# sun-huangqingbo/multiplexed-image-annotator

Measured on AMD Instinct MI355X. Metric: cells/sec annotated (whole node), higher is better.
Workload: dtype f16

## Files before the change

multiplexed-image-annotator_amd/_lib.py:

```python
from __future__ import annotations

import ctypes
import os
from ctypes import POINTER, c_char_p, c_double, c_float, c_int32, c_int64, c_uint32, c_uint64, c_void_p

HERE = os.path.dirname(os.path.abspath(__file__))
LIB_PATH = os.path.join(HERE, "libribca_hip.so")
if os.environ.get("RIBCA_LIB"):
    LIB_PATH = os.environ["RIBCA_LIB"] if os.path.isabs(os.environ["RIBCA_LIB"]) else os.path.join(HERE, os.environ["RIBCA_LIB"])

TEST_LIB_PATH = LIB_PATH[:-3] + "_test.so"

_lib = None
_test_lib = None

SIGNATURES = {
    "ribca_version": (c_int32, []),
    "ribca_last_error": (c_char_p, []),
    "ribca_mask_minmax": (c_int32, [c_void_p, c_int64, c_void_p, c_void_p]),
    "ribca_label_table": (c_int32, [c_void_p, c_int32, c_int32, c_int32, c_void_p, c_void_p, c_void_p]),
    "ribca_channel_min": (c_int32, [c_void_p, c_int32, c_int64, c_void_p, c_void_p]),
    "ribca_extract_patches": (c_int32, [c_void_p, c_int32, c_int32, c_int32, c_void_p, c_void_p, c_void_p, c_void_p, c_void_p, c_int32,
                                        c_void_p, c_void_p, c_void_p]),
    "ribca_extract_patches_scaled": (c_int32, [c_void_p, c_int32, c_int32, c_int32, c_void_p, c_void_p, c_void_p, c_void_p, c_void_p, c_int32,
# ... 148 lines not shown
                                            c_void_p, c_int32, c_void_p]),
    "ribca_test_gemm_fold": (c_int32, [c_int32, c_void_p, c_int32, c_void_p, c_int32, c_int32, c_int32, c_int32, c_void_p, c_void_p,
                                       c_void_p, c_void_p, c_int32, c_void_p]),
    "ribca_test_qkv_attention_fold": (c_int32, [c_void_p, c_int32, c_void_p, c_int32, c_int32, c_int32, c_int32, c_void_p, c_void_p,
                                                c_void_p, c_void_p, c_void_p, c_void_p, c_void_p, c_int32, c_void_p]),
    "ribca_test_gemm_duo_gelu": (c_int32, [c_void_p, c_int32, c_void_p, c_int32, c_int32, c_int32, c_int32, c_void_p, c_void_p, c_void_p,
                                           c_void_p, c_void_p, c_int32, c_void_p]),
    "ribca_test_cell_attention": (c_int32, [c_void_p, c_int32, c_void_p, c_int32, c_int32, c_int32, c_void_p, c_void_p, c_void_p, c_void_p, c_int32,
                                            c_void_p]),
    "ribca_test_cell_mlp_image_bytes": (c_int64, [c_int32]),
    "ribca_test_cell_mlp": (c_int32, [c_void_p, c_int32, c_void_p, c_void_p, c_void_p, c_void_p, c_void_p, c_void_p, c_void_p, c_void_p, c_int32,
                                      c_void_p, c_int32, c_void_p, c_int32, c_int32, c_void_p]),
    "ribca_test_cls_attention_cell_tile": (c_int32, []),
    "ribca_test_cls_attention": (c_int32, [c_void_p, c_int32, c_void_p, c_int32, c_void_p, c_void_p, c_int32, c_int32, c_void_p, c_void_p, c_void_p,
                                           c_int32, c_void_p]),
    "ribca_test_qkv_attention_tokens": (c_int32, [c_int32, c_void_p, c_int32, c_void_p, c_int32, c_int32, c_int32, c_int32, c_int32, c_int32, c_void_p,
                                                  c_void_p, c_void_p, c_void_p, c_void_p, c_void_p, c_void_p, c_int32, c_void_p]),
    "ribca_test_attention_v_elems": (c_int64, [c_int32, c_int32, c_int32, c_int32]),
    "ribca_gemm_padded_n": (c_int32, [c_int32]),
}


class RibcaError(RuntimeError):
    pass


class _Library:

    def __init__(self, handle):
        self._handle = handle
# ... 72 lines not shown
```

multiplexed-image-annotator_amd/build.py:

```python
from __future__ import annotations

import concurrent.futures
import os
import subprocess
import sys

HERE = os.path.dirname(os.path.abspath(__file__))
CSRC = os.path.join(HERE, "csrc")
LIB = os.path.join(HERE, "libribca_hip.so")
LIB_TEST = os.path.join(HERE, "libribca_hip_test.so")
TEST_SOURCES = ["ribca_test_api.hip"]
EXPORTS = os.path.join(CSRC, "exports.map")
SOURCES = ["gemm_split16.hip", "gemm_duo.hip", "gemm_mx.hip", "attention.hip", "cell_attention.hip", "cell_mlp.hip", "cls_attention.hip", "vit_misc.hip", "preprocess.hip", "preprocess_scaled.hip", "vote.hip", "colorize.hip", "knn.hip", "umap.hip", "hdbscan.hip", "regions.hip", "spectral.hip", "scatter.hip", "celltype_stats.hip", "perm.hip", "enrichment.hip", "autocorr.hip", "local_autocorr.hip", "cooccurrence.hip", "nearest.hip", "contact.hip", "morphology.hip", "intensities.hip", "expand.hip", "components.hip", "outlines.hip", "overlap.hip", "localization.hip", "normalize.hip", "ribca_api.hip"]
HEADERS = ["ribca_common.h", "ribca_kernels.h", "ribca_scratch.h", "ribca_perm.h", "ribca_rowtable.h", "ribca_cellbox.h", "ribca_status.h", "ribca_internal.h", "gemm_epi.h", os.path.join("..", "..", "include", "ribca_hip.h"),
           os.path.join("..", "..", "include", "ribca_hip_test.h")]
FLAGS = ["-O3", "--offload-arch=gfx950", "-fPIC", "-std=c++17", "-Wall", "-Wno-unused-function", "-fvisibility=hidden", "-fvisibility-inlines-hidden",
         "-fno-slp-vectorize"]


def source_fingerprint() -> str:
    import hashlib
    h = hashlib.sha256()
    for name in sorted(SOURCES + TEST_SOURCES) + sorted(HEADERS):
        path = os.path.normpath(os.path.join(CSRC, name))
        h.update(os.path.basename(path).encode() + b"\0")
        with open(path, "rb") as f:
            h.update(f.read())
    h.update(" ".join(FLAGS).encode())
# ... 60 lines not shown
```

multiplexed-image-annotator_amd/csrc/ribca_api.hip:

```cpp
#include <hip/hip_runtime.h>

#include <cmath>
#include <cstdarg>
#include <cstdlib>
#include <cstdio>
#include <cstring>
#include <string>
#include <vector>

#include "../../include/ribca_hip.h"
#include "ribca_common.h"
#include "ribca_internal.h"
#include "ribca_kernels.h"
#include "ribca_scratch.h"
#include "ribca_status.h"

using namespace ribca;

namespace {

int fail(const std::string& msg) { return api_fail(msg.c_str()); }
int hip_fail(hipError_t e, const char* what) { return api_hip_fail(e, what); }

inline int round_up(int v, int m) { return (v + m - 1) / m * m; }
// ... 69 lines not shown
}

struct BlockW {
  const float *ln1w, *ln1b, *qkvb, *projb, *ln2w, *ln2b, *fc1b, *fc2b;
  const uint16_t *qkvw, *projw, *fc1w, *fc2w;
  const uint16_t* qkvwf = nullptr;
  const uint16_t* fc1wf;
  const uint16_t *projwf = nullptr, *fc2wf = nullptr;
  const float *qkvc = nullptr, *qkvb2 = nullptr, *fc1c = nullptr, *fc1b2 = nullptr;
  const uint16_t* fc2mxh = nullptr; const unsigned char* fc2mxx = nullptr;
  const uint16_t *qkvmxh = nullptr, *fc1mxh = nullptr; const unsigned char *qkvmxx = nullptr, *fc1mxx = nullptr;
  const uint16_t* mlpimg = nullptr;
};

bool env_on(const char* name) { return !(getenv(name) && atoi(getenv(name)) == 0); }
struct Switches { bool mx, mxz, cell_attn, cell_mlp, cls_attn; };
const Switches& switches() {
  static const Switches sw = {env_on("RIBCA_MX"), env_on("RIBCA_MXZ"), env_on("RIBCA_CELL_ATTN"), env_on("RIBCA_CELL_MLP"), env_on("RIBCA_CLS_ATTN")};
  return sw;
}
bool mx_on(int D) { return switches().mx && (4 * D) % 128 == 0 && gemm_mx_supported(D, 4 * D); }
bool mx_z_on(int D) { return switches().mxz && mx_on(D) && D % 192 == 0; }

struct BlockPath {
  bool fold, mx_fc2, mx_z, cell_attn, cell_mlp, cls_attn;
  BlockPath precise() const { return {fold, false, false, cell_attn, cell_mlp, cls_attn}; }
  bool qkv_mx3() const { return mx_z && !cell_attn; }
  bool qkv_buffers() const { return !(cell_attn && cls_attn); }
};
BlockPath block_path(const AttnGeom& a, bool fold) {
  const bool cell_attn = fold && switches().cell_attn && cell_attention_supported(a.D, a.H, a.T);
  return {fold, fold && mx_on(a.D), fold && mx_z_on(a.D), cell_attn, cell_attn && switches().cell_mlp && cell_mlp_supported(a.D),
          fold && switches().cls_attn && cls_attention_supported(a.D, a.H, a.T)};
}

struct ribca_vit {
  int D, C, K, depth, Dp;
  BlockPath path;
  char* arena = nullptr;
  size_t arena_bytes = 0;
  const float *cls, *pos, *pe_b, *norm_w, *norm_b, *head_w, *head_b;
  const float* pe_w;
  std::vector<BlockW> layers;
};

struct ribca_mae {
  int L, enc_depth, dec_depth;
  BlockPath enc_path, dec_path;
// ... 113 lines not shown
      launch_mx_pack_w(L.fc1w, 2 * Dp, 4 * D, Dp, Kz, const_cast<uint16_t*>(L.fc1mxh), const_cast<unsigned char*>(L.fc1mxx), s);
    }
    if (path.cell_mlp) launch_cell_mlp_pack(L.projw, L.fc1w, L.fc2w, D, const_cast<uint16_t*>(L.mlpimg), s);
  }
};
int64_t block_params(int64_t d) { return 2 * d + 3 * d * d + 3 * d + d * d + d + 2 * d + 4 * d * d + 4 * d + 4 * d * d + d; }

struct BlockWs {
  float* z; uint16_t* xa; uint16_t* q; uint16_t* k; uint16_t* vt; uint16_t* h;
  size_t qk_bytes, vt_bytes, xa_bytes;
  uint16_t* zps = nullptr; float2* part = nullptr; float2* rs = nullptr;
  MxAct zmx = MxAct{nullptr, nullptr, nullptr, 0, 0};
  size_t zmx_rows = 0;
  float *cls_g = nullptr, *cls_y = nullptr;
};
BlockWs carve_blocks(Carver& c, int cells, const AttnGeom& a, const BlockPath& p) {
  BlockWs w;
  const size_t Mc = (size_t)cells * a.T;
  const int Dp = round_up(a.D, 32);
  if (p.fold) {
    w.z = nullptr;
    w.zps = c.take<uint16_t>(Mc * 2 * Dp);
    w.part = c.take<float2>((p.cell_mlp ? (size_t)cells : Mc) * gemm_resid_part_rows(a.D));
    w.rs = c.take<float2>(Mc);
    if (p.mx_z) {
      const int Kz = round_up(a.D, 128);
      w.zmx.hi = c.take<uint16_t>(Mc * Kz);
      w.zmx.l8 = c.take<unsigned char>(Mc * Kz);
      w.zmx.sc = c.take<unsigned char>(Mc * (Kz / 32));
      w.zmx.Kp = Kz;
      w.zmx_rows = Mc;
    }
  } else {
    w.z = c.take<float>(Mc * a.D);
  }
  w.xa_bytes = Mc * 2 * Dp * sizeof(uint16_t);
  w.xa = c.take<uint16_t>(Mc * 2 * Dp);
  w.q = w.k = w.vt = nullptr;
  w.qk_bytes = w.vt_bytes = 0;
  if (p.qkv_buffers()) {
    const size_t qk = (size_t)cells * a.H * a.TP * 2 * a.hdq;
    w.qk_bytes = qk * sizeof(uint16_t);
    w.q = c.take<uint16_t>(qk);
    w.k = c.take<uint16_t>(qk);
    const size_t vt = attention_v_elems(a, cells);
    w.vt_bytes = vt * sizeof(uint16_t);
    w.vt = c.take<uint16_t>(vt);
  }
  const size_t cls_elems = p.cls_attn ? cls_attention_scratch_elems(cells, a.D) : 0;
  if (p.cls_attn && !p.qkv_buffers()) {
    w.cls_g = c.take<float>(cls_elems);
    w.cls_y = c.take<float>(cls_elems);
  }
  w.h = c.take<uint16_t>((p.cell_mlp ? (size_t)cells : Mc) * 2 * 4 * a.D);
  if (p.cls_attn && p.qkv_buffers()) {
    w.cls_g = reinterpret_cast<float*>(w.h);
    w.cls_y = w.cls_g + cls_elems;
  }
  return w;
}
int zero_pads(const BlockWs& w, const BlockPath& p, hipStream_t s) {
  HIP_TRY(hipMemsetAsync(w.xa, 0, w.xa_bytes, s));
  if (p.fold) HIP_TRY(hipMemsetAsync(w.zps, 0, w.xa_bytes, s));
  if (p.qkv_buffers()) {
    HIP_TRY(hipMemsetAsync(w.q, 0, w.qk_bytes, s));
    HIP_TRY(hipMemsetAsync(w.k, 0, w.qk_bytes, s));
    HIP_TRY(hipMemsetAsync(w.vt, 0, w.vt_bytes, s));
  }
  if (p.mx_z) {
// ... 88 lines not shown
      launch_ln_finalize(w.part, sg.tiles, Mc, sg.bn, D, w.rs, s);
    }
    return;
  }
  {
    ProfScope ps(P_FC1, s);
    GemmArgs g{w.zps, ld_x, L.fc1w, ld_x, Mc, 4 * D, Dp, L.fc1b2, L.fc1wf};
    launch_gemm_gelu_ln(g, w.rs, L.fc1c, w.h, ld_h, s);
  }
  {
    ProfScope ps(P_FC2, s);
    GemmArgs g{w.h, ld_h, L.fc2w, ld_h, Mc, D, 4 * D, L.fc2b, L.fc2wf};
    resid_ps_and_stats(g, w, ld_x, D, true, 1, s);
  }
}
void run_last_block_cls_fold(const BlockW& L, const BlockWs& w, int cells, const AttnGeom& a, const BlockPath& p, hipStream_t s) {
  const int D = a.D, Dp = round_up(D, 32), ld_x = 2 * Dp, ld_h = 2 * 4 * D, Mc = cells * a.T;
  const float scale = 1.0f / sqrtf((float)a.hd);
  if (p.cls_attn) {
    { ProfScope ps(P_QKV, s); launch_cls_attn_qg(w.zps, ld_x, L.qkvw, ld_x, L.qkvb2, w.rs, cells, D, scale, w.cls_g, s); }
    {
      ProfScope ps(P_ATTN, s);
      launch_cls_attn_ybar(w.zps, ld_x, w.rs, w.cls_g, cells, D, w.cls_y, s);
      launch_cls_attn_out(w.cls_y, L.qkvw, ld_x, L.qkvb2, cells, D, w.xa, ld_x, s);
    }
  } else {
    {
      ProfScope ps(P_QKV, s);
      GemmArgs gkv{w.zps, ld_x, L.qkvw + (size_t)D * ld_x, ld_x, Mc, 2 * D, Dp, L.qkvb2 + D};
      launch_gemm_qkv_ln(gkv, w.rs, L.qkvc + D, w.q, w.k, w.vt, a, scale, s, D, 0, 1);
      GemmArgs gq{w.zps, a.T * ld_x, L.qkvw, ld_x, cells, D, Dp, L.qkvb2};
      launch_gemm_qkv_ln(gq, w.rs, L.qkvc, w.q, w.k, w.vt, a, scale, s, 0, 1, a.T);
    }
    { ProfScope ps(P_ATTN, s); launch_attention(w.q, w.k, w.vt, w.xa, ld_x, cells, a, s, 1); }
  }
  {
    ProfScope ps(P_PROJ, s);
    GemmArgs g{w.xa, a.T * ld_x, L.projw, ld_x, cells, D, Dp, L.projb};
    resid_ps_and_stats(g, w, a.T * ld_x, D, true, a.T, s);
// ... 36 lines not shown
  const int64_t d = D;
  return d + (int64_t)kTokens * d + d * C * 16 + d + (int64_t)depth * block_params(d) + 2 * d + (int64_t)K * d + K;
}

int ribca_vit_create(const float* blob, int64_t blob_len, int32_t D, int32_t C, int32_t K, int32_t depth, void* stream, ribca_vit_t** out) {
  if (!out) return fail("ribca_vit_create: out is NULL");
  *out = nullptr;
  if (D <= 0 || D % 48 != 0 || D > 768) return fail("ribca_vit_create: D must be a multiple of 48 and <= 768");
  if (C <= 0 || C > 64 || K <= 0 || K > 16 || depth <= 0) return fail("ribca_vit_create: bad C/K/depth");
  if (!attention_supported(make_attn_geom(D, kHeads, kTokens))) return fail("ribca_vit_create: unsupported head dimension");
  if (blob_len != ribca_vit_blob_len(D, C, K, depth)) return fail("ribca_vit_create: blob length does not match (D, C, K, depth)");
  hipStream_t s = (hipStream_t)stream;
  ribca_vit* m = new ribca_vit();
  m->D = D; m->C = C; m->K = K; m->depth = depth;
  m->Dp = round_up(D, 32);
  m->path = block_path(make_attn_geom(D, kHeads, kTokens), true);
  m->arena_bytes = layout(m, nullptr);
  hipError_t e = hipMalloc((void**)&m->arena, m->arena_bytes);
  if (e != hipSuccess) { delete m; return hip_fail(e, "hipMalloc(weights)"); }
  layout(m, m->arena);
  BlobReader r{blob, s};
  r.copy(m->cls, D);
  r.copy(m->pos, (size_t)kTokens * D);
  r.copy(m->pe_w, (size_t)D * 16 * C);
  r.copy(m->pe_b, D);
  for (auto& L : m->layers) r.block(L, D, m->path);
  r.copy(m->norm_w, D); r.copy(m->norm_b, D);
  r.copy(m->head_w, (size_t)K * D); r.copy(m->head_b, K);
  e = r.err != hipSuccess ? r.err : hipGetLastError();
  if (e != hipSuccess) { ribca_vit_destroy(m); return hip_fail(e, "weight packing"); }
  if (api_finish() != 0) { ribca_vit_destroy(m); return 1; }
// ... 44 lines not shown
      ProfScope ps(P_EMBED, s);
      launch_embed_ps(patches + (size_t)c0 * c_img * 1600, c_img, src_chan, m->C, m->pe_w, m->pe_b, m->pos, w.zps, ld_z, D, bc, s);
    }
    {
      ProfScope ps(P_OTHER, s);
      launch_cls_rows_ps(w.zps, ld_z, m->cls, m->pos, D, bc, kTokens, s);
    }
    { ProfScope ps(P_LN, s); launch_row_stats_ps(w.zps, ld_z, bc * kTokens, D, w.rs, true, s); }
    if (path.qkv_mx3() && n_whole > 0) {
      ProfScope ps(P_OTHER, s);
      MxAct zmx = w.zmx;
      zmx.M = bc * kTokens;
      launch_mx_pack_act(w.zps, ld_z, bc * kTokens, m->Dp, zmx, s);
    }
    for (size_t li = 0; li < n_whole; ++li) run_block_fold(m->layers[li], w, bc, geom, path, path.qkv_mx3() && li + 1 < n_whole, s);
    run_last_block_cls_fold(m->layers.back(), w, bc, geom, path, s);
    {
      ProfScope ps(P_HEAD, s);
      launch_head_softmax_ps(w.zps, ld_z, m->norm_w, m->norm_b, m->head_w, m->head_b, probs + (size_t)c0 * m->K, D, m->K, bc, s);
    }
  }
  RIBCA_FINISH();
  return 0;
}
int ribca_vit_forward(const ribca_vit_t* m, const float* patches, int32_t c_img, const int32_t* src_chan, int32_t n_cells, float* probs,
                      void* workspace, int64_t workspace_bytes, int32_t chunk_cells, void* stream) {
  if (!m) return fail("ribca_vit_forward: model is NULL");
  return vit_forward_impl(m, m->path, patches, c_img, src_chan, n_cells, probs, workspace, workspace_bytes, chunk_cells, stream);
}
int ribca_vit_forward_precise(const ribca_vit_t* m, const float* patches, int32_t c_img, const int32_t* src_chan, int32_t n_cells, float* probs,
                              void* workspace, int64_t workspace_bytes, int32_t chunk_cells, void* stream) {
  if (!m) return fail("ribca_vit_forward: model is NULL");
// ... 379 lines not shown
```

multiplexed-image-annotator_amd/csrc/ribca_internal.h:

```cpp
#pragma once
#include <stdint.h>

#include "ribca_kernels.h"
#include "ribca_status.h"

#define RIBCA_INTERNAL_VERSION 6005

#define RIBCA_INTERNAL_FUNCS(X)                                                                                                              \
  X(api_finish) X(api_fail) X(mx_wh_bytes) X(mx_wx_bytes) X(gemm_padded_n) X(gemm_resid_bn) X(gemm_resid_tiles) X(gemm_resid_part_rows)      \
  X(gemm_mx_supported) X(cell_attention_supported) X(make_attn_geom) X(launch_pack_wf)                                                      \
  X(launch_pack_weight) X(launch_pack_weight_fold) X(launch_mx_pack_w) X(launch_mx_pack_act) X(launch_layernorm_ps) X(launch_row_stats_ps)   \
  X(launch_ln_finalize) X(launch_gemm_resid) X(launch_gemm_gelu) X(launch_gemm_qkv) X(launch_gemm_qkv_ln) X(launch_gemm_gelu_ln)             \
  X(launch_gemm_gelu_mx) X(launch_gemm_resid_ps) X(launch_gemm_mx_resid) X(launch_gemm_mx_qkv_ln) X(launch_gemm_mx_gelu) X(launch_attention) \
  X(launch_cell_qkv_attention) X(cell_mlp_supported) X(cell_mlp_image_bytes) X(launch_cell_mlp_pack) X(launch_cell_mlp)                     \
  X(cls_attention_supported) X(cls_attention_cell_tile) X(launch_cls_attn_qg) X(launch_cls_attn_ybar) X(launch_cls_attn_out)           \
  X(attention_supported) X(attention_v_elems)

namespace ribca {
struct InternalTable {
  int32_t version;
  int32_t n_funcs;
#define RIBCA_X(name) decltype(&ribca::name) name;
  RIBCA_INTERNAL_FUNCS(RIBCA_X)
#undef RIBCA_X
};
}
```

multiplexed-image-annotator_amd/csrc/ribca_kernels.h:

```cpp
#pragma once
#include <hip/hip_runtime.h>
#include <stdint.h>

namespace ribca {

int gemm_pick_bn(int N);
int gemm_padded_n(int N);

struct GemmArgs {
  const uint16_t* A; int lda;
  const uint16_t* W; int ldw;
  int M, N, Kp;
  const float* bias;
  const uint16_t* WF = nullptr;
};
void launch_pack_wf(const uint16_t* W, int ldw, int Np, int Kp, uint16_t* WF, hipStream_t s);
void launch_gemm_resid(const GemmArgs& g, float* z, int ldz, hipStream_t s);
void launch_gemm_gelu(const GemmArgs& g, uint16_t* out, int ldo, hipStream_t s);
struct ResidStatGeom { int tiles, bn; };
struct MxAct { uint16_t* hi; unsigned char* l8; unsigned char* sc; int Kp; int M; };
ResidStatGeom launch_gemm_resid_ps(const GemmArgs& g, uint16_t* z, int ldz, float2* part, const float2* prev, int prev_stride, hipStream_t s,
                                   bool force_duo = false, const MxAct* zmx = nullptr);
int gemm_resid_tiles(int N);
int gemm_resid_bn(int N);
// ... 35 lines not shown
                               uint16_t* out, int ldo, int cells, int D, float scale, hipStream_t s);

bool cell_mlp_supported(int D);
size_t cell_mlp_image_bytes(int D);
void launch_cell_mlp_pack(const uint16_t* projw, const uint16_t* fc1w, const uint16_t* fc2w, int D, uint16_t* img, hipStream_t s);
void launch_cell_mlp(const uint16_t* xa, int ldx, const uint16_t* img, const float* projb, const float* fc1c, const float* fc1b2, const float* fc2b,
                     uint16_t* z, int ldz, float2* rs, int M, int D, hipStream_t s);

bool cls_attention_supported(int D, int H, int T);
int cls_attention_cell_tile();
size_t cls_attention_scratch_elems(int cells, int D);
void launch_cls_attn_qg(const uint16_t* z, int ldz, const uint16_t* W, int ldw, const float* bias2, const float2* rowstat, int cells, int D,
                        float scale, float* g, hipStream_t s);
void launch_cls_attn_ybar(const uint16_t* z, int ldz, const float2* rowstat, const float* g, int cells, int D, float* yb, hipStream_t s);
void launch_cls_attn_out(const float* yb, const uint16_t* W, int ldw, const float* bias2, int cells, int D, uint16_t* out, int ldo, hipStream_t s);

void launch_layernorm_ps(const float* z, int ldz, const float* gamma, const float* beta, uint16_t* out, int ldo, int M, int D,
                         hipStream_t s);
void launch_cls_rows(float* z, int ldz, const float* cls, const float* pos, int D, int cells, int tokens_per_cell, hipStream_t s);
void launch_layernorm_gather_ps(const float* z, int ldz, const float* gamma, const float* beta, uint16_t* out, int ldo, int cells, int T,
                                int S, const int* sel, int D, hipStream_t s);
void launch_layernorm_gather_ps_from_ps(const uint16_t* z_ps, int ldz, const float* gamma, const float* beta, uint16_t* out, int ldo, int cells,
                                        int T, int S, const int* sel, int D, hipStream_t s);
void launch_rows_to_ps(const float* src, int K, uint16_t* out, int ldo, int Kp, int cells, int T, int S, const int* sel, hipStream_t s);
void launch_fill_rows(float* z, int ldz, const float* a, const float* table, int D, int cells, int T, int S, const int* sel, hipStream_t s);
void launch_pack_weight(const float* w, int N, int K, uint16_t* out, int Np, int Kp, hipStream_t s);
void launch_embed_ps(const float* patches, int c_img, const int* src_chan, int C, const float* w, const float* bias, const float* pos,
                     uint16_t* z, int ldz, int D, int cells, hipStream_t s);
void launch_cls_rows_ps(uint16_t* z, int ldz, const float* cls, const float* pos, int D, int cells, int tokens_per_cell, hipStream_t s);
void launch_head_softmax_ps(const uint16_t* z, int ldz, const float* gamma, const float* beta, const float* hw, const float* hb,
// ... 63 lines not shown
```

multiplexed-image-annotator_amd/csrc/ribca_test_api.hip:

```cpp
#include <hip/hip_runtime.h>

#include <cmath>
#include <cstdint>
#include <cstdlib>
#include <string>

#include <utility>

#include "../../include/ribca_hip.h"
#include "../../include/ribca_hip_test.h"
#include "ribca_common.h"
#include "ribca_internal.h"

using ribca::AttnGeom;
using ribca::GemmArgs;
using ribca::kHeads;
using ribca::kTokens;
using ribca::MxAct;
using ribca::MxWeight;
using ribca::ResidStatGeom;

namespace {
const ribca::InternalTable* table() {
  static const ribca::InternalTable* t = static_cast<const ribca::InternalTable*>(ribca_internal_table(RIBCA_INTERNAL_VERSION));
// ... 271 lines not shown
}
int32_t ribca_test_cls_attention_cell_tile(void) { if (table() == nullptr) return 0; return cls_attention_cell_tile(); }
int ribca_test_cls_attention(const uint16_t* z_ps, int32_t ld, const uint16_t* W, int32_t ldw, const float* bias2, const float* rowstat,
                             int32_t cells, int32_t D, float* g, float* ybar, uint16_t* out, int32_t ldo, void* stream) {
  RIBCA_NEED_TABLE();
  if (!cls_attention_supported(D, kHeads, kTokens)) return fail("ribca_test_cls_attention: D must be 144, 288, 384 or 576");
  if (!z_ps || !W || !bias2 || !rowstat || !g || !ybar || !out || cells < 0) return fail("ribca_test_cls_attention: NULL buffer");
  const float scale = 1.0f / sqrtf((float)(D / kHeads));
  const float2* rs = reinterpret_cast<const float2*>(rowstat);
  launch_cls_attn_qg(z_ps, ld, W, ldw, bias2, rs, cells, D, scale, g, (hipStream_t)stream);
  launch_cls_attn_ybar(z_ps, ld, rs, g, cells, D, ybar, (hipStream_t)stream);
  launch_cls_attn_out(ybar, W, ldw, bias2, cells, D, out, ldo, (hipStream_t)stream);
  RIBCA_FINISH();
  return 0;
}
int ribca_test_qkv_attention(const uint16_t* A, int32_t lda, const uint16_t* W, int32_t ldw, int32_t cells, int32_t D, int32_t Kp,
                             const float* bias, uint16_t* q, uint16_t* k, uint16_t* vt, uint16_t* out, int32_t ldo, void* stream) {
  RIBCA_NEED_TABLE();
  const AttnGeom a = make_attn_geom(D, kHeads, kTokens);
  GemmArgs g{A, lda, W, ldw, cells * kTokens, 3 * D, Kp, bias};
  launch_gemm_qkv(g, q, k, vt, a, 1.0f / sqrtf((float)a.hd), (hipStream_t)stream);
  launch_attention(q, k, vt, out, ldo, cells, a, (hipStream_t)stream, 0);
  RIBCA_FINISH();
  return 0;
}
int64_t ribca_test_attention_v_elems(int32_t D, int32_t H, int32_t T, int32_t cells) {
  if (table() == nullptr || H <= 0 || T <= 0 || cells < 0) return 0;
  return (int64_t)attention_v_elems(make_attn_geom(D, H, T), cells);
}
int ribca_test_qkv_attention_tokens(int32_t fold, const uint16_t* a_or_z_ps, int32_t lda, const uint16_t* W, int32_t ldw, int32_t cells, int32_t D, int32_t H,
// ... 21 lines not shown
```

Measured before the change: 17660.

## Fuse last-block CLS tail (V-proj, proj, LN, MLP, head softmax) into one kernel

Adds a cls_tail kernel that handles the final transformer block for the CLS token in a single launch. It chains the V output projection, attention projection with residual, layernorm, the chunked fc1/GELU/fc2 MLP with residual, and the final norm/head softmax. Each workgroup processes a 16-cell tile kept in LDS. This is meant to remove the separate launches and the global-memory round trips between those stages for the CLS rows. In exchange it brings a large-LDS kernel with limited occupancy and split-f16 MFMA products, and it only applies to supported D and K values.

```diff
diff --git a/multiplexed-image-annotator_amd/_lib.py b/multiplexed-image-annotator_amd/_lib.py
--- a/multiplexed-image-annotator_amd/_lib.py
+++ b/multiplexed-image-annotator_amd/_lib.py
@@ -186,6 +186,14 @@
     "ribca_test_cls_attention_cell_tile": (c_int32, []),
     "ribca_test_cls_attention": (c_int32, [c_void_p, c_int32, c_void_p, c_int32, c_void_p, c_void_p, c_int32, c_int32, c_void_p, c_void_p, c_void_p,
                                            c_int32, c_void_p]),
+    "ribca_test_cls_attention_out": (c_int32, [c_void_p, c_void_p, c_int32, c_void_p, c_int32, c_int32, c_void_p, c_int32, c_void_p]),
+    "ribca_test_cls_tail_supported": (c_int32, [c_int32, c_int32]),
+    "ribca_test_cls_tail_cell_tile": (c_int32, []),
+    "ribca_test_cls_tail": (c_int32, [c_void_p, c_void_p, c_int32, c_void_p, c_void_p, c_void_p, c_void_p, c_void_p, c_void_p, c_void_p, c_void_p,
+                                      c_void_p, c_void_p, c_void_p, c_void_p, c_void_p, c_void_p, c_void_p, c_int32, c_int32, c_int32, c_int32,
+                                      c_void_p, c_void_p, c_void_p]),
+    "ribca_test_cls_tail_wf_elems": (c_int64, [c_int32]),
+    "ribca_test_head_softmax": (c_int32, [c_void_p, c_int32, c_void_p, c_void_p, c_void_p, c_void_p, c_int32, c_int32, c_int32, c_void_p, c_void_p]),
     "ribca_test_qkv_attention_tokens": (c_int32, [c_int32, c_void_p, c_int32, c_void_p, c_int32, c_int32, c_int32, c_int32, c_int32, c_int32, c_void_p,
                                                   c_void_p, c_void_p, c_void_p, c_void_p, c_void_p, c_void_p, c_int32, c_void_p]),
     "ribca_test_attention_v_elems": (c_int64, [c_int32, c_int32, c_int32, c_int32]),
diff --git a/multiplexed-image-annotator_amd/build.py b/multiplexed-image-annotator_amd/build.py
--- a/multiplexed-image-annotator_amd/build.py
+++ b/multiplexed-image-annotator_amd/build.py
@@ -11,7 +11,7 @@
 LIB_TEST = os.path.join(HERE, "libribca_hip_test.so")
 TEST_SOURCES = ["ribca_test_api.hip"]
 EXPORTS = os.path.join(CSRC, "exports.map")
-SOURCES = ["gemm_split16.hip", "gemm_duo.hip", "gemm_mx.hip", "attention.hip", "cell_attention.hip", "cell_mlp.hip", "cls_attention.hip", "vit_misc.hip", "preprocess.hip", "preprocess_scaled.hip", "vote.hip", "colorize.hip", "knn.hip", "umap.hip", "hdbscan.hip", "regions.hip", "spectral.hip", "scatter.hip", "celltype_stats.hip", "perm.hip", "enrichment.hip", "autocorr.hip", "local_autocorr.hip", "cooccurrence.hip", "nearest.hip", "contact.hip", "morphology.hip", "intensities.hip", "expand.hip", "components.hip", "outlines.hip", "overlap.hip", "localization.hip", "normalize.hip", "ribca_api.hip"]
+SOURCES = ["gemm_split16.hip", "gemm_duo.hip", "gemm_mx.hip", "attention.hip", "cell_attention.hip", "cell_mlp.hip", "cls_attention.hip", "cls_tail.hip", "vit_misc.hip", "preprocess.hip", "preprocess_scaled.hip", "vote.hip", "colorize.hip", "knn.hip", "umap.hip", "hdbscan.hip", "regions.hip", "spectral.hip", "scatter.hip", "celltype_stats.hip", "perm.hip", "enrichment.hip", "autocorr.hip", "local_autocorr.hip", "cooccurrence.hip", "nearest.hip", "contact.hip", "morphology.hip", "intensities.hip", "expand.hip", "components.hip", "outlines.hip", "overlap.hip", "localization.hip", "normalize.hip", "ribca_api.hip"]
 HEADERS = ["ribca_common.h", "ribca_kernels.h", "ribca_scratch.h", "ribca_perm.h", "ribca_rowtable.h", "ribca_cellbox.h", "ribca_status.h", "ribca_internal.h", "gemm_epi.h", os.path.join("..", "..", "include", "ribca_hip.h"),
            os.path.join("..", "..", "include", "ribca_hip_test.h")]
 FLAGS = ["-O3", "--offload-arch=gfx950", "-fPIC", "-std=c++17", "-Wall", "-Wno-unused-function", "-fvisibility=hidden", "-fvisibility-inlines-hidden",
diff --git a/multiplexed-image-annotator_amd/csrc/cls_tail.hip b/multiplexed-image-annotator_amd/csrc/cls_tail.hip
--- /dev/null
+++ b/multiplexed-image-annotator_amd/csrc/cls_tail.hip
@@ -0,0 +1,379 @@
+#include <type_traits>
+
+#include "ribca_common.h"
+#include "ribca_kernels.h"
+
+namespace ribca {
+namespace {
+
+constexpr int kCT = 16;
+constexpr int kThreads = 512, kNW = kThreads / 64;
+constexpr float kEps = 1e-6f;
+
+template <int D>
+struct Geo {
+  static constexpr int Dp = (D + 31) / 32 * 32, HD = D / kHeads;
+  static constexpr int NKD = Dp / 32;
+  static constexpr int NS = D > 384 ? 4 : 2;
+  static constexpr int SL = 4 * D / NS, NKS = SL / 32;
+  static constexpr int OJobs = HD % 16 == 0 ? D / 16 : HD == 24 ? D / 12 : D / 8;
+  __device__ static constexpr int o_tile(int j) { return HD % 16 == 0 ? j : HD == 24 ? 3 * (j / 4) + (j % 4 + 1) / 2 : 3 * (j / 6) + (j % 6) / 2; }
+  __device__ static constexpr int o_head(int j) { return HD % 16 == 0 ? 16 * j / HD : HD == 24 ? 2 * (j / 4) + (j % 4) / 2 : 4 * (j / 6) + (j % 6 + 1) / 2; }
+  static constexpr int UD = NKD % 3 == 0 ? 3 : NKD;
+  static constexpr int RD = NKD % 3 == 0 ? 4 : 2;
+  static constexpr int RowX = 4 * Dp + 32;
+  static constexpr int RowH = 4 * SL + 32;
+  static constexpr int RowF = 4 * D + 16;
+  static constexpr int OffO = 0;
+  static constexpr int OffX = OffO + kCT * RowX;
+  static constexpr int OffH = OffX + kCT * RowX;
+  static constexpr int OffS = OffH + kCT * RowH;
+  static constexpr int OffC = OffS + kCT * 16;
+  static constexpr int CBv = 0, CBp = D, CB2 = 2 * D, CC1 = 3 * D, CB1 = 7 * D;
+  static constexpr int Lds = OffC + 11 * D * 4;
+  static_assert(Lds <= 160 * 1024, "one workgroup's LDS");
+  static_assert(RowF <= RowX && NKS % 3 == 0 && D % 16 == 0 && HD % 4 == 0 && (HD % 16 == 0 || HD == 24 || HD == 12), "cls_tail geometry");
+};
+
+struct WRaw { u32x4 h, l; };
+struct NoRaw {};
+struct YRaw { float4 a, b; };
+
+__device__ __forceinline__ f16x8 frag(const u32x4& v) { return __builtin_bit_cast(f16x8, v); }
+
+__device__ __forceinline__ void split8(const YRaw& y, f16x8& hi, f16x8& lo) {
+  const float v0[4] = {y.a.x, y.a.y, y.a.z, y.a.w}, v1[4] = {y.b.x, y.b.y, y.b.z, y.b.w};
+  uint2 h0, l0, h1, l1;
+  split4(v0, h0, l0);
+  split4(v1, h1, l1);
+  hi = frag(u32x4{h0.x, h0.y, h1.x, h1.y});
+  lo = frag(u32x4{l0.x, l0.y, l1.x, l1.y});
+}
+__device__ __forceinline__ void lds_ps_store4(char* row, int n, const uint2& hi, const uint2& lo) {
+  char* p = row + 2 * ps_off(n);
+  *reinterpret_cast<uint2*>(p) = hi;
+  *reinterpret_cast<uint2*>(p + 16) = lo;
+}
+__device__ __forceinline__ void lds_ps_load4(const char* row, int n, float v[4]) {
+  const char* p = row + 2 * ps_off(n);
+  const uint2 hi = *reinterpret_cast<const uint2*>(p), lo = *reinterpret_cast<const uint2*>(p + 16);
+  v[0] = f16lo_plus_f16lo(hi.x, lo.x);
+  v[1] = f16hi_plus_f16hi(hi.x, lo.x);
+  v[2] = f16lo_plus_f16lo(hi.y, lo.y);
+  v[3] = f16hi_plus_f16hi(hi.y, lo.y);
+}
+__device__ __forceinline__ double half_sum(double v) {
+#pragma unroll
+  for (int o = 16; o > 0; o >>= 1) v += __shfl_xor(v, o, 64);
+  return v;
+}
+__device__ __forceinline__ float half_sum(float v) {
+#pragma unroll
+  for (int o = 16; o > 0; o >>= 1) v += __shfl_xor(v, o, 64);
+  return v;
+}
+
+template <int NK, int U, int R, class Raw, class WRow, class AFetch, class AFrag, class Begin, class End>
+__device__ __forceinline__ void product(int n_jobs, int wave, WRow wrow, AFetch afetch, AFrag afrag, Begin begin, End end) {
+  static_assert(NK % U == 0, "chunks tile the K steps");
+  constexpr int CPT = NK / U;
+  const int rounds = (n_jobs + kNW - 1) / kNW, total = rounds * CPT;
+  auto job_at = [&](int round) { const int j = wave + kNW * round; return j < n_jobs ? j : wave; };
+  WRaw rw[R][U];
+  Raw ra[R][U];
+  int pr = 0, pc = 0;
+  auto fetch = [&](WRaw* w, Raw* a) {
+    const int j = job_at(pr);
+    const uint16_t* p = wrow(j) + pc * (U * 1024);
+#pragma unroll
+    for (int i = 0; i < U; ++i) {
+      w[i].h = *reinterpret_cast<const u32x4*>(p + i * 1024);
+      w[i].l = *reinterpret_cast<const u32x4*>(p + i * 1024 + 512);
+      a[i] = afetch(j, pc * U + i);
+    }
+    if (++pc == CPT) { pc = 0; ++pr; }
+  };
+#pragma unroll
+  for (int u = 0; u < R; ++u) fetch(rw[u], ra[u]);
+  int cr = 0, cc = 0;
+  f32x4 acc = f32x4{0.f, 0.f, 0.f, 0.f}, acc1 = acc, acc2 = acc, accl = acc;
+  for (int c = 0; c < total; c += R) {
+#pragma unroll
+    for (int u = 0; u < R; ++u) {
+      if (c + u < total) {
+        if (cc == 0) {
+          acc = begin(job_at(cr));
+          acc1 = acc2 = accl = f32x4{0.f, 0.f, 0.f, 0.f};
+        }
+#pragma unroll
+        for (int i = 0; i < U; ++i) {
+          f16x8 ah, al;
+          afrag(ra[u][i], cc * U + i, ah, al);
+          const f16x8 wh = frag(rw[u][i].h), wl = frag(rw[u][i].l);
+          accl = mfma_f16(wl, ah, accl);
+          accl = mfma_f16(wh, al, accl);
+          if (i % 3 == 0) acc = mfma_f16(wh, ah, acc);
+          else if (i % 3 == 1) acc1 = mfma_f16(wh, ah, acc1);
+          else acc2 = mfma_f16(wh, ah, acc2);
+        }
+        if (c + u + R < total) fetch(rw[u], ra[u]);
+        if (++cc == CPT) {
+          cc = 0;
+          if (wave + kNW * cr < n_jobs) end(wave + kNW * cr, ((acc + acc1) + acc2) + accl);
+          ++cr;
+        }
+      }
+    }
+  }
+}
+
+template <int D>
+__global__ __launch_bounds__(kThreads) void cls_tail_kernel(const ClsTailArgs a) {
+  typedef Geo<D> G;
+  constexpr int Dp = G::Dp, HD = G::HD, SL = G::SL;
+  constexpr int NKD = G::NKD, NK2 = 4 * D / 32;
+  extern __shared__ __attribute__((aligned(16))) char smem[];
+  const int tid = threadIdx.x, lane = tid & 63;
+  const int wave = __builtin_amdgcn_readfirstlane(tid >> 6);
+  const int r16 = lane & 15, g = lane >> 4;
+  const int c0 = blockIdx.x * kCT;
+  const int cellr = c0 + r16 < a.cells ? c0 + r16 : a.cells - 1;
+  char* const rowO = smem + G::OffO + r16 * G::RowX;
+  char* const rowX = smem + G::OffX + r16 * G::RowX;
+  char* const rowH = smem + G::OffH + r16 * G::RowH;
+  float* const rowF = reinterpret_cast<float*>(smem + G::OffO + r16 * G::RowF);
+  const float pm0 = a.rs[(size_t)cellr * a.rs_stride].y;
+
+  float* const cst = reinterpret_cast<float*>(smem + G::OffC);
+
+  if constexpr (Dp != D) {
+    for (int i = tid; i < 2 * kCT * G::RowX / 16; i += kThreads) reinterpret_cast<uint4*>(smem)[i] = uint4{0u, 0u, 0u, 0u};
+    __syncthreads();
+  }
+  for (int i = tid; i < kCT * (D / 8); i += kThreads) {
+    const int c = i / (D / 8), grp = i % (D / 8);
+    const int cell = c0 + c < a.cells ? c0 + c : a.cells - 1;
+    const u32x4* p = reinterpret_cast<const u32x4*>(a.z + (size_t)cell * a.z_stride + 16 * grp);
+    u32x4* q = reinterpret_cast<u32x4*>(smem + G::OffX + c * G::RowX + 32 * grp);
+    q[0] = p[0];
+    q[1] = p[1];
+  }
+  for (int i = tid; i < D / 4; i += kThreads) {
+    reinterpret_cast<float4*>(cst + G::CBv)[i] = reinterpret_cast<const float4*>(a.qkvb2 + 2 * D)[i];
+    reinterpret_cast<float4*>(cst + G::CBp)[i] = reinterpret_cast<const float4*>(a.projb)[i];
+    reinterpret_cast<float4*>(cst + G::CB2)[i] = reinterpret_cast<const float4*>(a.fc2b)[i];
+  }
+  for (int i = tid; i < D; i += kThreads) {
+    reinterpret_cast<float4*>(cst + G::CC1)[i] = reinterpret_cast<const float4*>(a.fc1c)[i];
+    reinterpret_cast<float4*>(cst + G::CB1)[i] = reinterpret_cast<const float4*>(a.fc1b2)[i];
+  }
+  __syncthreads();
+  auto lds_frag = [&](const char* row, int s, f16x8& hi, f16x8& lo) {
+    const u32x4* p = reinterpret_cast<const u32x4*>(row + (4 * s + g) * 32);
+    hi = frag(p[0]);
+    lo = frag(p[1]);
+  };
+  auto no_fetch = [](int, int) { return NoRaw{}; };
+
+  {
+    product<G::NKD, G::UD, 2, YRaw>(
+        G::OJobs, wave, [&](int j) { return a.qkvwf + (size_t)((2 * D / 16 + G::o_tile(j)) * NKD) * 1024 + 8 * lane; },
+        [&](int j, int s) {
+          const int k = 32 * s + 8 * g;
+          if (k >= D) return YRaw{float4{0.f, 0.f, 0.f, 0.f}, float4{0.f, 0.f, 0.f, 0.f}};
+          const float4* p = reinterpret_cast<const float4*>(a.yb + ((size_t)cellr * kHeads + G::o_head(j)) * D + k);
+          return YRaw{p[0], p[1]};
+        },
+        [&](const YRaw& y, int, f16x8& hi, f16x8& lo) { split8(y, hi, lo); },
+        [&](int) { return f32x4{0.f, 0.f, 0.f, 0.f}; },
+        [&](int j, const f32x4& acc) {
+          const int n = 16 * G::o_tile(j) + 4 * g;
+          if (n / HD != G::o_head(j)) return;
+          const float4 b4 = *reinterpret_cast<const float4*>(cst + G::CBv + n);
+          const float x[4] = {acc[0] + b4.x, acc[1] + b4.y, acc[2] + b4.z, acc[3] + b4.w};
+          uint2 hi, lo;
+          split4(x, hi, lo);
+          lds_ps_store4(rowO, n, hi, lo);
+        });
+  }
+  __syncthreads();
+
+  {
+    product<G::NKD, G::UD, G::RD, NoRaw>(
+        D / 16, wave, [&](int j) { return a.projwf + (size_t)(j * NKD) * 1024 + 8 * lane; }, no_fetch,
+        [&](const NoRaw&, int s, f16x8& hi, f16x8& lo) { lds_frag(rowO, s, hi, lo); },
+        [&](int) { return f32x4{0.f, 0.f, 0.f, 0.f}; },
+        [&](int j, const f32x4& acc) {
+          const float4 b4 = *reinterpret_cast<const float4*>(cst + G::CBp + 16 * j + 4 * g);
+          float zo[4];
+          lds_ps_load4(rowX, 16 * j + 4 * g, zo);
+          const float b[4] = {b4.x, b4.y, b4.z, b4.w};
+          float x[4];
+#pragma unroll
+          for (int r = 0; r < 4; ++r) x[r] = clamp_f16_range((float)((double)zo[r] + ((double)acc[r] + ((double)b[r] - (double)pm0))));
+          uint2 hi, lo;
+          split4_unit(x, hi, lo);
+          lds_ps_store4(rowX, 16 * j + 4 * g, hi, lo);
+        });
+  }
+  __syncthreads();
+
+  const int sc = tid >> 5, sl = tid & 31;
+  {
+    constexpr int NQ = D / 4, NI = (NQ + 31) / 32;
+    const char* row = smem + G::OffX + sc * G::RowX;
+    float v[NI][4];
+    double sum = 0.0;
+#pragma unroll
+    for (int i = 0; i < NI; ++i) {
+      v[i][0] = v[i][1] = v[i][2] = v[i][3] = 0.f;
+      if (sl + 32 * i < NQ) lds_ps_load4(row, 4 * (sl + 32 * i), v[i]);
+      sum += ((double)v[i][0] + (double)v[i][1]) + ((double)v[i][2] + (double)v[i][3]);
+    }
+    const double md = half_sum(sum) / (double)D;
+    double q = 0.0;
+#pragma unroll
+    for (int i = 0; i < NI; ++i) {
+      if (sl + 32 * i < NQ) {
+        const double d0 = v[i][0] - md, d1 = v[i][1] - md, d2 = v[i][2] - md, d3 = v[i][3] - md;
+        q += (d0 * d0 + d1 * d1) + (d2 * d2 + d3 * d3);
+      }
+    }
+    const float mean = (float)md, rstd = (float)(1.0 / sqrt(half_sum(q) / (double)D + (double)kEps));
+    if (sl == 0) *reinterpret_cast<float4*>(smem + G::OffS + sc * 16) = float4{rstd, -mean * rstd, mean, 0.f};
+  }
+  __syncthreads();
+  const float4 st = *reinterpret_cast<const float4*>(smem + G::OffS + r16 * 16);
+
+#pragma unroll 1
+  for (int q = 0; q < G::NS; ++q) {
+    {
+      product<G::NKD, G::UD, G::RD, NoRaw>(
+          SL / 16, wave, [&](int j) { return a.fc1wf + (size_t)((q * (SL / 16) + j) * NKD) * 1024 + 8 * lane; }, no_fetch,
+          [&](const NoRaw&, int s, f16x8& hi, f16x8& lo) { lds_frag(rowX, s, hi, lo); },
+          [&](int) { return f32x4{0.f, 0.f, 0.f, 0.f}; },
+          [&](int j, const f32x4& acc) {
+            const int n = q * SL + 16 * j + 4 * g;
+            const float4 c4 = *reinterpret_cast<const float4*>(cst + G::CC1 + n), b4 = *reinterpret_cast<const float4*>(cst + G::CB1 + n);
+            const float c[4] = {c4.x, c4.y, c4.z, c4.w}, b[4] = {b4.x, b4.y, b4.z, b4.w};
+            float x[4];
+#pragma unroll
+            for (int r = 0; r < 4; ++r) x[r] = gelu_erf1(fmaf(st.x, acc[r], fmaf(st.y, c[r], b[r])));
+            uint2 hi, lo;
+            split4(x, hi, lo);
+            lds_ps_store4(rowH, 16 * j + 4 * g, hi, lo);
+          });
+    }
+    __syncthreads();
+    {
+      product<G::NKS, 3, 4, NoRaw>(
+          D / 16, wave, [&](int j) { return a.fc2wf + (size_t)(j * NK2 + q * G::NKS) * 1024 + 8 * lane; }, no_fetch,
+          [&](const NoRaw&, int s, f16x8& hi, f16x8& lo) { lds_frag(rowH, s, hi, lo); },
+          [&](int j) {
+            const int n = 16 * j + 4 * g;
+            if (q == 0) return f32x4{0.f, 0.f, 0.f, 0.f};
+            const float4 p = *reinterpret_cast<const float4*>(rowF + n);
+            return f32x4{p.x, p.y, p.z, p.w};
+          },
+          [&](int j, const f32x4& acc) {
+            const int n = 16 * j + 4 * g;
+            float x[4] = {acc[0], acc[1], acc[2], acc[3]};
+            if (q == G::NS - 1) {
+              float x1[4];
+              lds_ps_load4(rowX, n, x1);
+              const float4 b4 = *reinterpret_cast<const float4*>(cst + G::CB2 + n);
+              const float b[4] = {b4.x, b4.y, b4.z, b4.w};
+#pragma unroll
+              for (int r = 0; r < 4; ++r) x[r] = clamp_f16_range((float)((double)x1[r] + ((double)acc[r] + ((double)b[r] - (double)st.z))));
+            }
+            *reinterpret_cast<float4*>(rowF + n) = float4{x[0], x[1], x[2], x[3]};
+          });
+    }
+    __syncthreads();
+  }
+
+  {
+    constexpr int NI = (D + 31) / 32;
+    const int cell = c0 + sc;
+    const bool ok = cell < a.cells;
+    const float* row = reinterpret_cast<const float*>(smem + G::OffO + sc * G::RowF);
+    float x[NI];
+    double sum = 0.0;
+#pragma unroll
+    for (int i = 0; i < NI; ++i) {
+      const int d = sl + 32 * i;
+      x[i] = d < D ? row[d] : 0.f;
+      sum += (double)x[i];
+    }
+    if (a.x2_out != nullptr && ok) {
+#pragma unroll
+      for (int i = 0; i < NI; ++i)
+        if (sl + 32 * i < D) a.x2_out[(size_t)cell * D + sl + 32 * i] = x[i];
+    }
+    const double md = half_sum(sum) / (double)D;
+    double q = 0.0;
+#pragma unroll
+    for (int i = 0; i < NI; ++i)
+      if (sl + 32 * i < D) { const double dd = x[i] - md; q += dd * dd; }
+    const double rstd = 1.0 / sqrt(half_sum(q) / (double)D + (double)kEps);
+    float* const yhi = reinterpret_cast<float*>(smem + G::OffO + sc * G::RowF);
+    float* const ylo = reinterpret_cast<float*>(smem + G::OffX + sc * G::RowF);
+#pragma unroll
+    for (int i = 0; i < NI; ++i) {
+      const int d = sl + 32 * i;
+      if (d < D) {
+        const double y = ((double)x[i] - md) * rstd * (double)a.norm_w[d] + (double)a.norm_b[d];
+        const float h = (float)y;
+        yhi[d] = h;
+        ylo[d] = (float)(y - (double)h);
+      }
+    }
+    __syncthreads();
+    const int k = sl & 15, half = sl >> 4, kk = k < a.K ? k : a.K - 1;
+    const float4* hw = reinterpret_cast<const float4*>(a.head_w + (size_t)kk * D + half * (D / 2));
+    const float4* yh = reinterpret_cast<const float4*>(yhi + half * (D / 2));
+    const float4* yl = reinterpret_cast<const float4*>(ylo + half * (D / 2));
+    double p0 = 0.0, p1 = 0.0, p2 = 0.0, p3 = 0.0;
+#pragma unroll 6
+    for (int i = 0; i < D / 8; ++i) {
+      const float4 w = hw[i], u = yh[i], v = yl[i];
+      p0 = fma((double)u.x + (double)v.x, (double)w.x, p0);
+      p1 = fma((double)u.y + (double)v.y, (double)w.y, p1);
+      p2 = fma((double)u.z + (double)v.z, (double)w.z, p2);
+      p3 = fma((double)u.w + (double)v.w, (double)w.w, p3);
+    }
+    const double part = (p0 + p1) + (p2 + p3);
+    const double logit = (part + __shfl_xor(part, 16, 64)) + (double)a.head_b[kk];
+    double mx = k < a.K ? logit : -__builtin_inf();
+#pragma unroll
+    for (int o = 8; o > 0; o >>= 1) mx = fmax(mx, __shfl_xor(mx, o, 64));
+    const double e = k < a.K ? exp(logit - mx) : 0.0;
+    double den = e;
+#pragma unroll
+    for (int o = 8; o > 0; o >>= 1) den += __shfl_xor(den, o, 64);
+    if (ok && half == 0 && k < a.K) a.probs[(size_t)cell * a.K + k] = (float)(e / den);
+  }
+}
+
+template <int D>
+void launch_width(const ClsTailArgs& a, hipStream_t s) {
+  static unsigned long long attr_done = 0ull;
+  if (!ensure_dynamic_lds(reinterpret_cast<const void*>(cls_tail_kernel<D>), Geo<D>::Lds, attr_done)) return;
+  hipLaunchKernelGGL(cls_tail_kernel<D>, dim3((unsigned)((a.cells + kCT - 1) / kCT)), dim3(kThreads), Geo<D>::Lds, s, a);
+}
+
+}
+
+bool cls_tail_supported(int D, int K) { return (D == 144 || D == 288 || D == 384 || D == 576) && K >= 1 && K <= 16; }
+int cls_tail_cell_tile() { return kCT; }
+
+void launch_cls_tail(const ClsTailArgs& a, int D, hipStream_t s) {
+  if (a.cells <= 0) return;
+  if (!cls_tail_supported(D, a.K)) { launch_error("cls_tail: no form for D = %d, K = %d", D, a.K); return; }
+  if (D == 144) launch_width<144>(a, s);
+  else if (D == 288) launch_width<288>(a, s);
+  else if (D == 384) launch_width<384>(a, s);
+  else launch_width<576>(a, s);
+}
+
+}
diff --git a/multiplexed-image-annotator_amd/csrc/ribca_api.hip b/multiplexed-image-annotator_amd/csrc/ribca_api.hip
--- a/multiplexed-image-annotator_amd/csrc/ribca_api.hip
+++ b/multiplexed-image-annotator_amd/csrc/ribca_api.hip
@@ -107,24 +107,26 @@
 };
 
 bool env_on(const char* name) { return !(getenv(name) && atoi(getenv(name)) == 0); }
-struct Switches { bool mx, mxz, cell_attn, cell_mlp, cls_attn; };
+struct Switches { bool mx, mxz, cell_attn, cell_mlp, cls_attn, cls_tail; };
 const Switches& switches() {
-  static const Switches sw = {env_on("RIBCA_MX"), env_on("RIBCA_MXZ"), env_on("RIBCA_CELL_ATTN"), env_on("RIBCA_CELL_MLP"), env_on("RIBCA_CLS_ATTN")};
+  static const Switches sw = {env_on("RIBCA_MX"), env_on("RIBCA_MXZ"), env_on("RIBCA_CELL_ATTN"), env_on("RIBCA_CELL_MLP"), env_on("RIBCA_CLS_ATTN"),
+                              env_on("RIBCA_CLS_TAIL")};
   return sw;
 }
 bool mx_on(int D) { return switches().mx && (4 * D) % 128 == 0 && gemm_mx_supported(D, 4 * D); }
 bool mx_z_on(int D) { return switches().mxz && mx_on(D) && D % 192 == 0; }
 
 struct BlockPath {
-  bool fold, mx_fc2, mx_z, cell_attn, cell_mlp, cls_attn;
-  BlockPath precise() const { return {fold, false, false, cell_attn, cell_mlp, cls_attn}; }
+  bool fold, mx_fc2, mx_z, cell_attn, cell_mlp, cls_attn, cls_tail;
+  BlockPath precise() const { return {fold, false, false, cell_attn, cell_mlp, cls_attn, cls_tail}; }
   bool qkv_mx3() const { return mx_z && !cell_attn; }
   bool qkv_buffers() const { return !(cell_attn && cls_attn); }
 };
-BlockPath block_path(const AttnGeom& a, bool fold) {
+BlockPath block_path(const AttnGeom& a, bool fold, int K = 0) {
   const bool cell_attn = fold && switches().cell_attn && cell_attention_supported(a.D, a.H, a.T);
-  return {fold, fold && mx_on(a.D), fold && mx_z_on(a.D), cell_attn, cell_attn && switches().cell_mlp && cell_mlp_supported(a.D),
-          fold && switches().cls_attn && cls_attention_supported(a.D, a.H, a.T)};
+  const bool cls_attn = fold && switches().cls_attn && cls_attention_supported(a.D, a.H, a.T);
+  return {fold, fold && mx_on(a.D), fold && mx_z_on(a.D), cell_attn, cell_attn && switches().cell_mlp && cell_mlp_supported(a.D), cls_attn,
+          cls_attn && K > 0 && switches().cls_tail && cls_tail_supported(a.D, K)};
 }
 
 struct ribca_vit {
@@ -268,6 +270,7 @@
   size_t zmx_rows = 0;
   float *cls_g = nullptr, *cls_y = nullptr;
 };
+size_t tail_rows(const BlockPath& p, int cells, size_t Mc) { return !p.cell_mlp ? Mc : p.cls_tail ? 0 : (size_t)cells; }
 BlockWs carve_blocks(Carver& c, int cells, const AttnGeom& a, const BlockPath& p) {
   BlockWs w;
   const size_t Mc = (size_t)cells * a.T;
@@ -275,7 +278,7 @@
   if (p.fold) {
     w.z = nullptr;
     w.zps = c.take<uint16_t>(Mc * 2 * Dp);
-    w.part = c.take<float2>((p.cell_mlp ? (size_t)cells : Mc) * gemm_resid_part_rows(a.D));
+    w.part = c.take<float2>(tail_rows(p, cells, Mc) * gemm_resid_part_rows(a.D));
     w.rs = c.take<float2>(Mc);
     if (p.mx_z) {
       const int Kz = round_up(a.D, 128);
@@ -306,7 +309,7 @@
     w.cls_g = c.take<float>(cls_elems);
     w.cls_y = c.take<float>(cls_elems);
   }
-  w.h = c.take<uint16_t>((p.cell_mlp ? (size_t)cells : Mc) * 2 * 4 * a.D);
+  w.h = c.take<uint16_t>(tail_rows(p, cells, Mc) * 2 * 4 * a.D);
   if (p.cls_attn && p.qkv_buffers()) {
     w.cls_g = reinterpret_cast<float*>(w.h);
     w.cls_y = w.cls_g + cls_elems;
@@ -425,7 +428,8 @@
     resid_ps_and_stats(g, w, ld_x, D, true, 1, s);
   }
 }
-void run_last_block_cls_fold(const BlockW& L, const BlockWs& w, int cells, const AttnGeom& a, const BlockPath& p, hipStream_t s) {
+void run_last_block_cls_fold(const ribca_vit* m, const BlockWs& w, int cells, const AttnGeom& a, const BlockPath& p, float* probs, hipStream_t s) {
+  const BlockW& L = m->layers.back();
   const int D = a.D, Dp = round_up(D, 32), ld_x = 2 * Dp, ld_h = 2 * 4 * D, Mc = cells * a.T;
   const float scale = 1.0f / sqrtf((float)a.hd);
   if (p.cls_attn) {
@@ -433,7 +437,14 @@
     {
       ProfScope ps(P_ATTN, s);
       launch_cls_attn_ybar(w.zps, ld_x, w.rs, w.cls_g, cells, D, w.cls_y, s);
-      launch_cls_attn_out(w.cls_y, L.qkvw, ld_x, L.qkvb2, cells, D, w.xa, ld_x, s);
+      if (!p.cls_tail) launch_cls_attn_out(w.cls_y, L.qkvw, ld_x, L.qkvb2, cells, D, w.xa, ld_x, s);
+    }
+    if (p.cls_tail) {
+      ProfScope ps(P_FC2, s);
+      const ClsTailArgs t{w.cls_y, w.zps, (size_t)a.T * ld_x, w.rs, a.T, L.qkvwf, L.qkvb2, L.projwf, L.projb, L.fc1wf, L.fc1c, L.fc1b2, L.fc2wf, L.fc2b,
+                          m->norm_w, m->norm_b, m->head_w, m->head_b, probs, nullptr, m->K, cells};
+      launch_cls_tail(t, D, s);
+      return;
     }
   } else {
     {
@@ -500,7 +511,7 @@
   ribca_vit* m = new ribca_vit();
   m->D = D; m->C = C; m->K = K; m->depth = depth;
   m->Dp = round_up(D, 32);
-  m->path = block_path(make_attn_geom(D, kHeads, kTokens), true);
+  m->path = block_path(make_attn_geom(D, kHeads, kTokens), true, K);
   m->arena_bytes = layout(m, nullptr);
   hipError_t e = hipMalloc((void**)&m->arena, m->arena_bytes);
   if (e != hipSuccess) { delete m; return hip_fail(e, "hipMalloc(weights)"); }
@@ -575,8 +586,8 @@
       launch_mx_pack_act(w.zps, ld_z, bc * kTokens, m->Dp, zmx, s);
     }
     for (size_t li = 0; li < n_whole; ++li) run_block_fold(m->layers[li], w, bc, geom, path, path.qkv_mx3() && li + 1 < n_whole, s);
-    run_last_block_cls_fold(m->layers.back(), w, bc, geom, path, s);
-    {
+    run_last_block_cls_fold(m, w, bc, geom, path, probs + (size_t)c0 * m->K, s);
+    if (!path.cls_tail) {
       ProfScope ps(P_HEAD, s);
       launch_head_softmax_ps(w.zps, ld_z, m->norm_w, m->norm_b, m->head_w, m->head_b, probs + (size_t)c0 * m->K, D, m->K, bc, s);
     }
diff --git a/multiplexed-image-annotator_amd/csrc/ribca_internal.h b/multiplexed-image-annotator_amd/csrc/ribca_internal.h
--- a/multiplexed-image-annotator_amd/csrc/ribca_internal.h
+++ b/multiplexed-image-annotator_amd/csrc/ribca_internal.h
@@ -4,7 +4,7 @@
 #include "ribca_kernels.h"
 #include "ribca_status.h"
 
-#define RIBCA_INTERNAL_VERSION 6005
+#define RIBCA_INTERNAL_VERSION 6006
 
 #define RIBCA_INTERNAL_FUNCS(X)                                                                                                              \
   X(api_finish) X(api_fail) X(mx_wh_bytes) X(mx_wx_bytes) X(gemm_padded_n) X(gemm_resid_bn) X(gemm_resid_tiles) X(gemm_resid_part_rows)      \
@@ -14,7 +14,7 @@
   X(launch_gemm_gelu_mx) X(launch_gemm_resid_ps) X(launch_gemm_mx_resid) X(launch_gemm_mx_qkv_ln) X(launch_gemm_mx_gelu) X(launch_attention) \
   X(launch_cell_qkv_attention) X(cell_mlp_supported) X(cell_mlp_image_bytes) X(launch_cell_mlp_pack) X(launch_cell_mlp)                     \
   X(cls_attention_supported) X(cls_attention_cell_tile) X(launch_cls_attn_qg) X(launch_cls_attn_ybar) X(launch_cls_attn_out)           \
-  X(attention_supported) X(attention_v_elems)
+  X(cls_tail_supported) X(cls_tail_cell_tile) X(launch_cls_tail) X(launch_head_softmax_ps) X(attention_supported) X(attention_v_elems)
 
 namespace ribca {
 struct InternalTable {
diff --git a/multiplexed-image-annotator_amd/csrc/ribca_kernels.h b/multiplexed-image-annotator_amd/csrc/ribca_kernels.h
--- a/multiplexed-image-annotator_amd/csrc/ribca_kernels.h
+++ b/multiplexed-image-annotator_amd/csrc/ribca_kernels.h
@@ -73,6 +73,22 @@
                         float scale, float* g, hipStream_t s);
 void launch_cls_attn_ybar(const uint16_t* z, int ldz, const float2* rowstat, const float* g, int cells, int D, float* yb, hipStream_t s);
 void launch_cls_attn_out(const float* yb, const uint16_t* W, int ldw, const float* bias2, int cells, int D, uint16_t* out, int ldo, hipStream_t s);
+
+struct ClsTailArgs {
+  const float* yb;
+  const uint16_t* z; size_t z_stride;
+  const float2* rs; int rs_stride;
+  const uint16_t* qkvwf; const float* qkvb2;
+  const uint16_t* projwf; const float* projb;
+  const uint16_t* fc1wf; const float *fc1c, *fc1b2;
+  const uint16_t* fc2wf; const float* fc2b;
+  const float *norm_w, *norm_b, *head_w, *head_b;
+  float* probs; float* x2_out;
+  int K, cells;
+};
+bool cls_tail_supported(int D, int K);
+int cls_tail_cell_tile();
+void launch_cls_tail(const ClsTailArgs& a, int D, hipStream_t s);
 
 void launch_layernorm_ps(const float* z, int ldz, const float* gamma, const float* beta, uint16_t* out, int ldo, int M, int D,
                          hipStream_t s);
diff --git a/multiplexed-image-annotator_amd/csrc/ribca_test_api.hip b/multiplexed-image-annotator_amd/csrc/ribca_test_api.hip
--- a/multiplexed-image-annotator_amd/csrc/ribca_test_api.hip
+++ b/multiplexed-image-annotator_amd/csrc/ribca_test_api.hip
@@ -309,6 +309,56 @@
   RIBCA_FINISH();
   return 0;
 }
+int ribca_test_cls_attention_out(const float* ybar, const uint16_t* W, int32_t ldw, const float* bias2, int32_t cells, int32_t D, uint16_t* out,
+                                 int32_t ldo, void* stream) {
+  RIBCA_NEED_TABLE();
+  if (!cls_attention_supported(D, kHeads, kTokens)) return fail("ribca_test_cls_attention_out: D must be 144, 288, 384 or 576");
+  if (!ybar || !W || !bias2 || !out || cells < 0) return fail("ribca_test_cls_attention_out: NULL buffer");
+  launch_cls_attn_out(ybar, W, ldw, bias2, cells, D, out, ldo, (hipStream_t)stream);
+  RIBCA_FINISH();
+  return 0;
+}
+int32_t ribca_test_cls_tail_supported(int32_t D, int32_t K) { if (table() == nullptr) return 0; return cls_tail_supported(D, K) ? 1 : 0; }
+int64_t ribca_test_cls_tail_wf_elems(int32_t D) {
+  if (table() == nullptr) return 0;
+  const int Dp = round_up(D, 32);
+  return (int64_t)(gemm_padded_n(3 * D) + gemm_padded_n(D) + gemm_padded_n(4 * D)) * 2 * Dp + (int64_t)gemm_padded_n(D) * 2 * 4 * D;
+}
+int32_t ribca_test_cls_tail_cell_tile(void) { if (table() == nullptr) return 0; return cls_tail_cell_tile(); }
+int ribca_test_cls_tail(const float* ybar, const uint16_t* z_ps, int32_t ld, const float* rowstat, const uint16_t* qkvw, const float* qkvb2,
+                        const uint16_t* projw, const float* projb, const uint16_t* fc1w, const float* fc1c, const float* fc1b2, const uint16_t* fc2w,
+                        const float* fc2b, const float* norm_w, const float* norm_b, const float* head_w, const float* head_b, uint16_t* wf_scratch,
+                        int32_t pack, int32_t cells, int32_t D, int32_t K, float* probs, float* x2_out, void* stream) {
+  RIBCA_NEED_TABLE();
+  if (!cls_tail_supported(D, K)) return fail("ribca_test_cls_tail: D must be 144, 288, 384 or 576 and K in 1 .. 16");
+  if (!ybar || !z_ps || !rowstat || !qkvw || !qkvb2 || !projw || !projb || !fc1w || !fc1c || !fc1b2 || !fc2w || !fc2b || !norm_w || !norm_b ||
+      !head_w || !head_b || !wf_scratch || !probs || cells < 0)
+    return fail("ribca_test_cls_tail: NULL buffer");
+  if (ld < 2 * round_up(D, 32)) return fail("ribca_test_cls_tail: ld is smaller than a packed-split row");
+  const int Dp = round_up(D, 32);
+  const size_t n3 = (size_t)gemm_padded_n(3 * D) * 2 * Dp, n1 = (size_t)gemm_padded_n(D) * 2 * Dp, n4 = (size_t)gemm_padded_n(4 * D) * 2 * Dp;
+  uint16_t *qkvwf = wf_scratch, *projwf = qkvwf + n3, *fc1wf = projwf + n1, *fc2wf = fc1wf + n4;
+  if (pack) {
+    launch_pack_wf(qkvw, 2 * Dp, gemm_padded_n(3 * D), Dp, qkvwf, (hipStream_t)stream);
+    launch_pack_wf(projw, 2 * Dp, gemm_padded_n(D), Dp, projwf, (hipStream_t)stream);
+    launch_pack_wf(fc1w, 2 * Dp, gemm_padded_n(4 * D), Dp, fc1wf, (hipStream_t)stream);
+    launch_pack_wf(fc2w, 2 * 4 * D, gemm_padded_n(D), 4 * D, fc2wf, (hipStream_t)stream);
+  }
+  const ribca::ClsTailArgs a{ybar, z_ps, (size_t)kTokens * ld, reinterpret_cast<const float2*>(rowstat), kTokens, qkvwf, qkvb2, projwf, projb, fc1wf,
+                             fc1c, fc1b2, fc2wf, fc2b, norm_w, norm_b, head_w, head_b, probs, x2_out, K, cells};
+  launch_cls_tail(a, D, (hipStream_t)stream);
+  RIBCA_FINISH();
+  return 0;
+}
+int ribca_test_head_softmax(const uint16_t* z_ps, int32_t ld, const float* norm_w, const float* norm_b, const float* head_w, const float* head_b,
+                            int32_t cells, int32_t D, int32_t K, float* probs, void* stream) {
+  RIBCA_NEED_TABLE();
+  if (!z_ps || !norm_w || !norm_b || !head_w || !head_b || !probs || cells < 0) return fail("ribca_test_head_softmax: NULL buffer");
+  if (D <= 0 || D > 768 || K < 1 || K > 16) return fail("ribca_test_head_softmax: D must be in 1 .. 768 and K in 1 .. 16");
+  launch_head_softmax_ps(z_ps, ld, norm_w, norm_b, head_w, head_b, probs, D, K, cells, (hipStream_t)stream);
+  RIBCA_FINISH();
+  return 0;
+}
 int ribca_test_qkv_attention(const uint16_t* A, int32_t lda, const uint16_t* W, int32_t ldw, int32_t cells, int32_t D, int32_t Kp,
                              const float* bias, uint16_t* q, uint16_t* k, uint16_t* vt, uint16_t* out, int32_t ldo, void* stream) {
   RIBCA_NEED_TABLE();
```

New measurement: 17530. No clear change (-0.8%).
